# nianticlabs/implicit-depth

Hardware: AMD Instinct MI355X
Metric: frames/sec (BDModel.forward hot path, 512x384, 64 planes, 8-frame tuple = 1 current + 7 source views; third-party backbones excluded) (higher is better)
Workload: dtype f32

## Files before the change

### implicit-depth_amd/csrc/conv.hip

```cpp
#include <algorithm>
#include "conv_args.h"
#include "../../include/idh_ops.h"

using namespace idh_conv;

int idh_stem_op(const idh_op &op, hipStream_t st, bool launch);

namespace {

__device__ float g_zero_page[kZeroFloats];

thread_local bool t_dry_run = false;
thread_local int t_launches = 0;
#undef IDH_CHECK_LAUNCH
#define IDH_CHECK_LAUNCH()                                              \
    do {                                                                \
        if (!t_dry_run && hipGetLastError() != hipSuccess) return IDH_ELAUNCH; \
    } while (0)
#define IDH_LAUNCH(...)                         \
    do {                                        \
        if (t_dry_run) ++t_launches;            \
        else hipLaunchKernelGGL(__VA_ARGS__);   \
    } while (0)

// ... 694 lines not shown
        const int c4 = (int)(t & 3);
        long long r = t >> 2;
        const int co = (int)(r % Cout_pad);
        r /= Cout_pad;
        const int cq = (int)(r % (Cin_pad / 4));
        const int tap = (int)(r / (Cin_pad / 4));
        const int ci = cq * 4 + c4;
        float v = 0.f;
        if (ci < Cin && co < Cout) v = w[((size_t)co * Cin + ci) * taps + tap];
        dst[t] = v;
    }
}

__device__ __forceinline__ void upsample2_body(const float *__restrict__ in, float *__restrict__ out, int N, int H, int W, int C,
                                               int in_cs, int out_cs, unsigned blk, unsigned nblk) {
    const unsigned cq = (unsigned)C >> 2;
    const int Wo = 2 * W;
    const unsigned total = (unsigned)N * H * W * cq;
    constexpr float lo = 0.25f, hi = 0.75f;
    for (unsigned t = blk * 256u + threadIdx.x; t < total; t += nblk * 256u) {
        const unsigned q = t % cq;
        unsigned p = t / cq;
        const int ix = (int)(p % (unsigned)W);
        p /= (unsigned)W;
        const int iy = (int)(p % (unsigned)H);
        const int n = (int)(p / (unsigned)H);
        const int xm = max(ix - 1, 0), xp = min(ix + 1, W - 1);
        const int ym = max(iy - 1, 0), yp = min(iy + 1, H - 1);
        const float *b = in + (size_t)n * H * W * in_cs + 4 * q;
        const float *r0 = b + (size_t)ym * W * in_cs, *r1 = b + (size_t)iy * W * in_cs, *r2 = b + (size_t)yp * W * in_cs;
        float4 v[3][3];
        v[0][0] = *reinterpret_cast<const float4 *>(r0 + (size_t)xm * in_cs);
        v[0][1] = *reinterpret_cast<const float4 *>(r0 + (size_t)ix * in_cs);
        v[0][2] = *reinterpret_cast<const float4 *>(r0 + (size_t)xp * in_cs);
        v[1][0] = *reinterpret_cast<const float4 *>(r1 + (size_t)xm * in_cs);
        v[1][1] = *reinterpret_cast<const float4 *>(r1 + (size_t)ix * in_cs);
        v[1][2] = *reinterpret_cast<const float4 *>(r1 + (size_t)xp * in_cs);
        v[2][0] = *reinterpret_cast<const float4 *>(r2 + (size_t)xm * in_cs);
        v[2][1] = *reinterpret_cast<const float4 *>(r2 + (size_t)ix * in_cs);
        v[2][2] = *reinterpret_cast<const float4 *>(r2 + (size_t)xp * in_cs);
        float4 e[3], o[3];
#pragma unroll
        for (int r = 0; r < 3; ++r) {
            e[r].x = lo * v[r][0].x + hi * v[r][1].x; e[r].y = lo * v[r][0].y + hi * v[r][1].y;
            e[r].z = lo * v[r][0].z + hi * v[r][1].z; e[r].w = lo * v[r][0].w + hi * v[r][1].w;
            o[r].x = hi * v[r][1].x + lo * v[r][2].x; o[r].y = hi * v[r][1].y + lo * v[r][2].y;
            o[r].z = hi * v[r][1].z + lo * v[r][2].z; o[r].w = hi * v[r][1].w + lo * v[r][2].w;
        }
        float4 o00, o01, o10, o11;
        o00.x = lo * e[0].x + hi * e[1].x; o00.y = lo * e[0].y + hi * e[1].y; o00.z = lo * e[0].z + hi * e[1].z; o00.w = lo * e[0].w + hi * e[1].w;
        o01.x = lo * o[0].x + hi * o[1].x; o01.y = lo * o[0].y + hi * o[1].y; o01.z = lo * o[0].z + hi * o[1].z; o01.w = lo * o[0].w + hi * o[1].w;
        o10.x = hi * e[1].x + lo * e[2].x; o10.y = hi * e[1].y + lo * e[2].y; o10.z = hi * e[1].z + lo * e[2].z; o10.w = hi * e[1].w + lo * e[2].w;
        o11.x = hi * o[1].x + lo * o[2].x; o11.y = hi * o[1].y + lo * o[2].y; o11.z = hi * o[1].z + lo * o[2].z; o11.w = hi * o[1].w + lo * o[2].w;
        float *d = out + (((size_t)n * 2 * H + 2 * iy) * Wo + 2 * ix) * out_cs + 4 * q;
        *reinterpret_cast<float4 *>(d) = o00;
        *reinterpret_cast<float4 *>(d + out_cs) = o01;
        *reinterpret_cast<float4 *>(d + (size_t)Wo * out_cs) = o10;
        *reinterpret_cast<float4 *>(d + (size_t)Wo * out_cs + out_cs) = o11;
    }
}

__global__ __launch_bounds__(256) void upsample2_k(const float *__restrict__ in, float *__restrict__ out, int N, int H,
                                                   int W, int C, int in_cs, int out_cs) {
    upsample2_body(in, out, N, H, W, C, in_cs, out_cs, blockIdx.x, gridDim.x);
}

__global__ __launch_bounds__(256) void upsample2_nearest_k(const float *__restrict__ in, float *__restrict__ out, int N, int H,
                                                           int W, int C, int in_cs, int out_cs) {
    const int cq = C >> 2;
    const int Ho = 2 * H, Wo = 2 * W;
    const long long total = (long long)N * Ho * Wo * cq;
    for (long long t = blockIdx.x * 256ll + threadIdx.x; t < total; t += gridDim.x * 256ll) {
        const int q = (int)(t % cq);
        long long p = t / cq;
        const int x = (int)(p % Wo);
        p /= Wo;
        const int y = (int)(p % Ho);
        const int n = (int)(p / Ho);
        const float4 v = *reinterpret_cast<const float4 *>(in + (((size_t)n * H + (y >> 1)) * W + (x >> 1)) * in_cs + 4 * q);
        *reinterpret_cast<float4 *>(out + (((size_t)n * Ho + y) * Wo + x) * out_cs + 4 * q) = v;
    }
}

__global__ __launch_bounds__(256) void copy_nhwc_k(const float *__restrict__ in, float *__restrict__ out, long long npix, int C,
                                                   int in_cs, int out_cs) {
    const int cq = C >> 2;
    const long long total = npix * cq;
    for (long long t = blockIdx.x * 256ll + threadIdx.x; t < total; t += gridDim.x * 256ll) {
        const int q = (int)(t % cq);
        const long long p = t / cq;
        *reinterpret_cast<float4 *>(out + p * out_cs + 4 * q) = *reinterpret_cast<const float4 *>(in + p * in_cs + 4 * q);
    }
}

__device__ __forceinline__ void import_nchw_body(const float *__restrict__ src, float *__restrict__ dst, int C, int HW, int out_cs, int bx, int by, int img,
                                                 float (&tile)[32][65]) {
    const int p0 = bx * 64, c0 = by * 32;
    const float *s = src + (size_t)img * C * HW;
    float *d = dst + (size_t)img * HW * out_cs;
    for (int i = threadIdx.x; i < 64 * 32; i += 256) {
        const int p = i & 63, c = i >> 6;
        if (p0 + p < HW && c0 + c < C) tile[c][p] = s[(size_t)(c0 + c) * HW + p0 + p];
    }
    __syncthreads();
    for (int i = threadIdx.x; i < 64 * 32; i += 256) {
        const int c = i & 31, p = i >> 5;
        if (p0 + p < HW && c0 + c < C) d[(size_t)(p0 + p) * out_cs + c0 + c] = tile[c][p];
    }
}

__global__ __launch_bounds__(256) void import_nchw_k(const float *__restrict__ src, float *__restrict__ dst, int C,
                                                     int HW, int out_cs) {
    __shared__ float tile[32][65];
    import_nchw_body(src, dst, C, HW, out_cs, blockIdx.x, blockIdx.y, blockIdx.z, tile);
}

constexpr int kMaxImport = 8;
struct ImportGroupArgs {
    int n;
    unsigned start[kMaxImport + 1];
    struct { const float *src; float *dst; int C, HW, out_cs, nbx, nby; } d[kMaxImport];
};
__global__ __launch_bounds__(256) void import_nchw_group_k(const ImportGroupArgs g) {
    __shared__ float tile[32][65];
    int idx = 0;
    for (int i = 1; i < g.n; ++i)
        if (blockIdx.x >= g.start[i]) idx = i;
    const auto &m = g.d[idx];
    const unsigned local = blockIdx.x - g.start[idx];
    const int bx = (int)(local % (unsigned)m.nbx);
    const unsigned r = local / (unsigned)m.nbx;
    import_nchw_body(m.src, m.dst, m.C, m.HW, m.out_cs, bx, (int)(r % (unsigned)m.nby), (int)(r / (unsigned)m.nby), tile);
}

__global__ __launch_bounds__(256) void export_nchw_k(const float *__restrict__ src, float *__restrict__ dst, int C,
                                                     int HW, int in_cs) {
    __shared__ float tile[32][65];
    const int img = blockIdx.z;
    const int p0 = blockIdx.x * 64, c0 = blockIdx.y * 32;
    const float *s = src + (size_t)img * HW * in_cs;
    float *d = dst + (size_t)img * C * HW;
    for (int i = threadIdx.x; i < 64 * 32; i += 256) {
        const int c = i & 31, p = i >> 5;
        if (p0 + p < HW && c0 + c < C) tile[c][p] = s[(size_t)(p0 + p) * in_cs + c0 + c];
    }
    __syncthreads();
    for (int i = threadIdx.x; i < 64 * 32; i += 256) {
        const int p = i & 63, c = i >> 6;
        if (p0 + p < HW && c0 + c < C) d[(size_t)(c0 + c) * HW + p0 + p] = tile[c][p];
    }
}

constexpr int kPwCin = 64, kPwCout = 128, kPwTile = 64;
struct PwNchwArgs {
    const float *in, *w, *bias;
    float *out;
    int HW, out_cs, tiles_per_img;
    long long tiles;
};

__global__ __launch_bounds__(256, 4) void pointwise_nchw_k(const PwNchwArgs a) {
    constexpr int C16 = kPwCin / 16, NT = kPwCout / 16;
    __shared__ f32x4 sW[(kPwCin / 4) * kPwCout];
    {
        const f32x4 *g = reinterpret_cast<const f32x4 *>(a.w);
        for (int i = threadIdx.x; i < (kPwCin / 4) * kPwCout; i += 256) sW[i] = g[i];
    }
    __syncthreads();
    const int lane = threadIdx.x & 63;
    const int wave = __builtin_amdgcn_readfirstlane(threadIdx.x >> 6);
    const int ln = lane & 15, h = lane >> 4;

    const unsigned img_bytes = (unsigned)kPwCin * (unsigned)a.HW * 4u;
    auto load = [&](long long tile, f32x4 (&x)[C16]) {
        const int n = (int)(tile / a.tiles_per_img);
        const int p = (int)(tile - (long long)n * a.tiles_per_img) * kPwTile + 16 * wave + ln;
        const __amdgpu_buffer_rsrc_t rs = __builtin_amdgcn_make_buffer_rsrc(const_cast<float *>(a.in + (size_t)n * kPwCin * a.HW), 0, img_bytes, 0x00020000);
        const int voff = p < a.HW ? (4 * h * a.HW + p) * 4 : (int)0x7fffffff;
#pragma unroll
        for (int c = 0; c < C16; ++c)
#pragma unroll
            for (int e = 0; e < 4; ++e)
                x[c][e] = __builtin_bit_cast(float, __builtin_amdgcn_raw_buffer_load_b32(rs, voff, (16 * c + e) * a.HW * 4, 0));
    };
    auto compute = [&](long long tile, const f32x4 (&x)[C16]) {
        f32x4 acc[NT];
#pragma unroll
        for (int j = 0; j < NT; ++j) acc[j] = (f32x4){0.f, 0.f, 0.f, 0.f};
        int opaque = 0;
        asm volatile("" : "+s"(opaque));
        const f32x4 *sWt = sW + opaque;
#pragma unroll
        for (int c = 0; c < C16; ++c)
#pragma unroll
            for (int j = 0; j < NT; ++j) {
                const f32x4 A = sWt[(4 * c + h) * kPwCout + 16 * j + ln];
#pragma unroll
                for (int kk = 0; kk < 4; ++kk) acc[j] = __builtin_amdgcn_mfma_f32_16x16x4f32(A[kk], x[c][kk], acc[j], 0, 0, 0);
            }
        const int n = (int)(tile / a.tiles_per_img);
        const int p = (int)(tile - (long long)n * a.tiles_per_img) * kPwTile + 16 * wave + ln;
        if (p < a.HW) {
            float *o = a.out + ((size_t)n * a.HW + p) * a.out_cs + 4 * h;
#pragma unroll
            for (int j = 0; j < NT; ++j) {
                f32x4 v = acc[j];
                if (a.bias) v += *reinterpret_cast<const f32x4 *>(a.bias + 16 * j + 4 * h);
                *reinterpret_cast<f32x4 *>(o + 16 * j) = v;
            }
        }
    };
    f32x4 xa[C16], xb[C16];
    long long t = blockIdx.x;
    if (t >= a.tiles) return;
    load(t, xa);
    for (;;) {
        const long long t1 = t + gridDim.x;
        if (t1 < a.tiles) load(t1, xb);
        compute(t, xa);
        if (t1 >= a.tiles) break;
        const long long t2 = t1 + gridDim.x;
        if (t2 < a.tiles) load(t2, xa);
        compute(t1, xb);
        if (t2 >= a.tiles) break;
        t = t2;
    }
}

struct PwUpArgs {
    const float *in, *w, *bias, *low;
    float *out;
    int H, W, in_cs, low_cs, out_cs, tiles_per_img;
    long long tiles;
};

template <int C16, int NT>
__global__ __launch_bounds__(256) void pointwise_up_k(const PwUpArgs a) {
    constexpr int kCout = 16 * NT;
    extern __shared__ f32x4 sWu[];
    {
        const f32x4 *g = reinterpret_cast<const f32x4 *>(a.w);
        for (int i = threadIdx.x; i < 4 * C16 * kCout; i += 256) sWu[i] = g[i];
    }
    __syncthreads();
    const int lane = threadIdx.x & 63;
    const int wave = __builtin_amdgcn_readfirstlane(threadIdx.x >> 6);
    const int ln = lane & 15, h = lane >> 4;
    const int HW = a.H * a.W, Hl = a.H >> 1, Wl = a.W >> 1;
    for (long long tile = blockIdx.x; tile < a.tiles; tile += gridDim.x) {
        const int n = (int)(tile / a.tiles_per_img);
        const int p = (int)(tile - (long long)n * a.tiles_per_img) * kPwTile + 16 * wave + ln;
        const bool ok = p < HW;
        const int pc = ok ? p : 0;
        const float *ip = a.in + ((size_t)n * HW + pc) * a.in_cs + 4 * h;
        f32x4 x[C16];
#pragma unroll
        for (int c = 0; c < C16; ++c) x[c] = *reinterpret_cast<const f32x4 *>(ip + 16 * c);
        const int y = pc / a.W, xq = pc - y * a.W;
        const int iy = y >> 1, ix = xq >> 1;
        int y0, y1, x0, x1;
        float hy0, hy1, wx0, wx1;
        if (y & 1) { y0 = iy; y1 = min(iy + 1, Hl - 1); hy0 = 0.75f; hy1 = 0.25f; }
        else { y0 = max(iy - 1, 0); y1 = iy; hy0 = 0.25f; hy1 = 0.75f; }
        if (xq & 1) { x0 = ix; x1 = min(ix + 1, Wl - 1); wx0 = 0.75f; wx1 = 0.25f; }
        else { x0 = max(ix - 1, 0); x1 = ix; wx0 = 0.25f; wx1 = 0.75f; }
        const float *lb = a.low + (size_t)n * Hl * Wl * a.low_cs + 4 * h;
        const float *t00 = lb + ((size_t)y0 * Wl + x0) * a.low_cs, *t01 = lb + ((size_t)y0 * Wl + x1) * a.low_cs;
        const float *t10 = lb + ((size_t)y1 * Wl + x0) * a.low_cs, *t11 = lb + ((size_t)y1 * Wl + x1) * a.low_cs;
        f32x4 acc[NT];
#pragma unroll
        for (int j = 0; j < NT; ++j) acc[j] = a.bias ? *reinterpret_cast<const f32x4 *>(a.bias + 16 * j + 4 * h) : (f32x4){0.f, 0.f, 0.f, 0.f};
        int opaque = 0;
        asm volatile("" : "+s"(opaque));
        const f32x4 *sWt = sWu + opaque;
#pragma unroll
        for (int c = 0; c < C16; ++c)
#pragma unroll
            for (int j = 0; j < NT; ++j) {
                const f32x4 A = sWt[(4 * c + h) * kCout + 16 * j + ln];
#pragma unroll
                for (int kk = 0; kk < 4; ++kk) acc[j] = __builtin_amdgcn_mfma_f32_16x16x4f32(A[kk], x[c][kk], acc[j], 0, 0, 0);
            }
        if (ok) {
            float *o = a.out + ((size_t)n * HW + p) * a.out_cs + 4 * h;
#pragma unroll
            for (int j = 0; j < NT; ++j) {
                const f32x4 p00 = *reinterpret_cast<const f32x4 *>(t00 + 16 * j), p01 = *reinterpret_cast<const f32x4 *>(t01 + 16 * j);
                const f32x4 p10 = *reinterpret_cast<const f32x4 *>(t10 + 16 * j), p11 = *reinterpret_cast<const f32x4 *>(t11 + 16 * j);
                f32x4 v;
#pragma unroll
                for (int e = 0; e < 4; ++e) v[e] = acc[j][e] + (hy0 * (wx0 * p00[e] + wx1 * p01[e]) + hy1 * (wx0 * p10[e] + wx1 * p11[e]));
                *reinterpret_cast<f32x4 *>(o + 16 * j) = v;
            }
        }
    }
}

__global__ __launch_bounds__(256) void pointwise_head_k(const float *__restrict__ in, const float *__restrict__ w,
                                                        const float *__restrict__ bias, float *__restrict__ out,
                                                        float *__restrict__ out_exp, long long M, int C, int in_cs) {
    for (long long m = blockIdx.x * 256ll + threadIdx.x; m < M; m += gridDim.x * 256ll) {
        const float4 *p = reinterpret_cast<const float4 *>(in + m * in_cs);
        const float4 *wv = reinterpret_cast<const float4 *>(w);
        float s = 0.f;
        for (int q = 0; q < (C >> 2); ++q) {
            const float4 a = p[q], b = wv[q];
            s = fmaf(a.x, b.x, s); s = fmaf(a.y, b.y, s); s = fmaf(a.z, b.z, s); s = fmaf(a.w, b.w, s);
        }
        const float v = s + (bias ? bias[0] : 0.f);
        out[m] = v;
        if (out_exp) out_exp[m] = expf(v);
    }
}

constexpr int kInChunk = 1024;

template <int SUB>
__global__ __launch_bounds__(1024) void instnorm_stats_k(const float *__restrict__ in, int cs, int C, int HW, int nchunks,
                                                         float *__restrict__ part) {
    extern __shared__ float red[];
    const int n = blockIdx.y, chunk = blockIdx.x;
    const int cq = C >> 2;
    const int q = threadIdx.x % cq;
    const int prow = threadIdx.x / cq, pstep = (int)blockDim.x / cq;
    const int rows = SUB * pstep;
    const int p0 = chunk * kInChunk, p1 = min(HW, p0 + kInChunk);
    const float4 pv = *reinterpret_cast<const float4 *>(in + (size_t)n * HW * cs + 4 * q);
    float s[SUB][4], ss[SUB][4];
#pragma unroll
    for (int u = 0; u < SUB; ++u)
#pragma unroll
        for (int e = 0; e < 4; ++e) s[u][e] = ss[u][e] = 0.f;
    for (int p = p0 + prow; p < p1; p += rows) {
#pragma unroll
        for (int u = 0; u < SUB; ++u) {
            const int pp = p + u * pstep;
            if (pp < p1) {
                const float4 v = *reinterpret_cast<const float4 *>(in + ((size_t)n * HW + pp) * cs + 4 * q);
                const float d0 = v.x - pv.x, d1 = v.y - pv.y, d2 = v.z - pv.z, d3 = v.w - pv.w;
                s[u][0] += d0; s[u][1] += d1; s[u][2] += d2; s[u][3] += d3;
                ss[u][0] = fmaf(d0, d0, ss[u][0]); ss[u][1] = fmaf(d1, d1, ss[u][1]); ss[u][2] = fmaf(d2, d2, ss[u][2]); ss[u][3] = fmaf(d3, d3, ss[u][3]);
            }
        }
    }
#pragma unroll
    for (int u = 0; u < SUB; ++u) {
        float *mine = red + ((size_t)(prow + u * pstep) * cq + q) * 8;
#pragma unroll
        for (int e = 0; e < 4; ++e) { mine[e] = s[u][e]; mine[4 + e] = ss[u][e]; }
    }
    __syncthreads();
    for (int t = threadIdx.x; t < 8 * cq; t += blockDim.x) {
        const int qq = t >> 3, e = t & 7;
        float a = 0.f;
        for (int r = 0; r < rows; ++r) a += red[(r * cq + qq) * 8 + e];
        part[((size_t)(n * nchunks + chunk) * 2 + (e >> 2)) * C + 4 * qq + (e & 3)] = a;
    }
}

__global__ __launch_bounds__(256) void instnorm_finalize_k(const float *__restrict__ part, const float *__restrict__ in, int cs, int C, int HW,
                                                           int nchunks, float *__restrict__ stats) {
    const int n = blockIdx.x;
    for (int c = threadIdx.x; c < C; c += 256) {
        float s = 0.f, ss = 0.f;
        for (int k = 0; k < nchunks; ++k) {
            const float *o = part + ((size_t)(n * nchunks + k) * 2) * C + c;
            s += o[0];
            ss += o[C];
        }
        const float ms = s / (float)HW;
        const float var = fmaxf(ss / (float)HW - ms * ms, 0.f);
        stats[(size_t)n * 2 * C + c] = in[(size_t)n * HW * cs + c] + ms;
        stats[(size_t)n * 2 * C + C + c] = 1.0f / sqrtf(var + 1e-5f);
    }
}

__global__ __launch_bounds__(256) void instnorm_apply_k(const float *__restrict__ in, int cs, float *__restrict__ out, int out_cs,
                                                        int C, int HW, long long total, const float *__restrict__ stats, int act,
// ... 332 lines not shown
                PreparedConv pcs[kMaxGroup];
                int kinds[kMaxGroup];
                int run = 0;
                for (int j = i; j < n && run < kMaxGroup; ++j) {
                    const idh_op &o = ops[j];
                    if (j > i && (op.group == 0 || o.group != op.group)) break;
                    PreparedConv &pc = pcs[run];
                    if (o.kind == IDH_OP_CONV) {
                        const int rc = prep_conv(o, pc);
                        if (rc != IDH_OK) return rc;
                        kinds[run] = level_kind(pc);
                    } else if (o.kind == IDH_OP_UPSAMPLE2) {
                        const int rc = check_upsample(o);
                        if (rc != IDH_OK) return rc;
                        const idh_conv_src &us = o.src[0];
                        pc = PreparedConv{};
                        ConvArgs &c = pc.la.c;
                        c.s[0].in = us.in; c.s[0].H = us.H; c.s[0].W = us.W; c.s[0].Cin = us.Cin; c.s[0].cs = us.cs;
                        c.out = o.out; c.out_cs = o.out_cs; c.M = o.N; c.S = 1;
                        pc.a = c;
                        const long long tot = (long long)o.N * 4 * us.H * us.W * (us.Cin >> 2);
                        const long long natural = idh_cdiv(tot, 256);
                        pc.blocks = (unsigned)std::min<long long>(idh_cdiv(tot / 4, 256), kLevelUpsampleBlocks);
                        kinds[run] = natural <= kLevelUpsampleNatural ? LV_UP2 : -1;
                    } else {
                        break;
                    }
                    ++run;
                }
                int cnt = 0;
                if (op.kind == IDH_OP_CONV && pcs[0].lds_rows == 4 && !pcs[0].norm && !pcs[0].s2) {
                    cnt = 1;
                    while (cnt < run && ops[i + cnt].kind == IDH_OP_CONV && pcs[cnt].lds_rows == 4 && pcs[cnt].nj == pcs[0].nj &&
                           (!pcs[cnt].up || pcs[0].nj == 4) && !pcs[cnt].norm && !pcs[cnt].s2)
                        ++cnt;
                }
                int mix = 0;
                while (mix < run && kinds[mix] >= 0 && pcs[mix].blocks <= kLevelMaxBlocks) ++mix;
                int wg = 0;
                if (op.kind == IDH_OP_CONV && pcs[0].lds_rows == 32) {
                    wg = 1;
                    while (wg < run && wg < wino_max_group() && ops[i + wg].kind == IDH_OP_CONV && pcs[wg].lds_rows == 32 &&
                           (pcs[wg].a.s[1].in != nullptr) == (pcs[0].a.s[1].in != nullptr))
                        ++wg;
                }
                int rc, used;
                if (wg > 1) {
                    if (t_dry_run) {
                        ++t_launches;
                        rc = IDH_OK;
                    } else {
                        const ConvArgs *as[kMaxGroup];
                        int ns[kMaxGroup];
                        for (int j = 0; j < wg; ++j) { as[j] = &pcs[j].a; ns[j] = pcs[j].n_img; }
                        rc = launch_conv_wino_group(as, ns, wg, st);
                        if (rc == IDH_EUNSUPPORTED) {
                            rc = IDH_OK;
                            for (int j = 0; j < wg && rc == IDH_OK; ++j) rc = launch_conv(pcs[j], st);
                        }
                    }
                    used = wg;
                } else if (mix > cnt && mix > 1) {
                    rc = launch_level(pcs, kinds, mix, st);
                    used = mix;
                } else if (cnt > 1) {
                    rc = launch_group(pcs, cnt, st);
                    used = cnt;
                } else if (op.kind == IDH_OP_CONV) {
                    rc = launch_conv(pcs[0], st);
                    if (rc == IDH_OK) rc = launch_reduces(pcs, 1, st);
                    used = 1;
                } else {
                    const long long quads = (long long)op.N * s.H * s.W * (s.Cin >> 2);
                    int grid = idh_cdiv(quads, 256);
                    if (grid > 32768) grid = 32768;
                    IDH_LAUNCH(upsample2_k, dim3(grid), dim3(256), 0, st, s.in, op.out, op.N, s.H, s.W, s.Cin, s.cs, op.out_cs);
                    IDH_CHECK_LAUNCH();
                    rc = IDH_OK;
                    used = 1;
                }
                if (rc != IDH_OK) return rc;
                i += used - 1;
                break;
            }
            case IDH_OP_UPSAMPLE2_NEAREST: {
                if (!s.in || !op.out || (s.Cin & 3) || (s.cs & 3) || (op.out_cs & 3) || op.N <= 0) return IDH_EINVAL;
                const long long tot = (long long)op.N * 4 * s.H * s.W * (s.Cin >> 2);
                int grid = idh_cdiv(tot, 256);
                if (grid > 8192) grid = 8192;
                IDH_LAUNCH(upsample2_nearest_k, dim3(grid), dim3(256), 0, st, s.in, op.out, op.N, s.H, s.W, s.Cin, s.cs, op.out_cs);
                IDH_CHECK_LAUNCH();
                break;
            }
            case IDH_OP_NCHW_TO_NHWC: {
                ImportGroupArgs g{};
                unsigned cursor = 0;
                int run = 0;
                for (int j = i; j < n && run < kMaxImport; ++j) {
                    const idh_op &o = ops[j];
                    if (o.kind != IDH_OP_NCHW_TO_NHWC || (j > i && (op.group == 0 || o.group != op.group))) break;
                    const idh_conv_src &os = o.src[0];
                    if (!os.in || !o.out || o.N <= 0 || o.N > 65535 || os.H <= 0 || os.W <= 0 || os.Cin <= 0) return IDH_EINVAL;
                    const int HWj = os.H * os.W;
                    const long long blocks = (long long)idh_cdiv(HWj, 64) * idh_cdiv(os.Cin, 32) * o.N;
                    if (blocks > kLevelMaxBlocks * 8ll || cursor + blocks >= (1ll << 31)) break;
                    g.d[run].src = os.in; g.d[run].dst = o.out; g.d[run].C = os.Cin; g.d[run].HW = HWj; g.d[run].out_cs = o.out_cs;
                    g.d[run].nbx = idh_cdiv(HWj, 64); g.d[run].nby = idh_cdiv(os.Cin, 32);
                    g.start[run] = cursor;
                    cursor += (unsigned)blocks;
                    ++run;
                }
                if (run > 1) {
                    g.n = run;
                    g.start[run] = cursor;
                    IDH_LAUNCH(import_nchw_group_k, dim3(cursor), dim3(256), 0, st, g);
                    IDH_CHECK_LAUNCH();
                    i += run - 1;
                    break;
                }
                if (!s.in || !op.out || op.N <= 0 || op.N > 65535) return IDH_EINVAL;
                const int HW = s.H * s.W;
                IDH_LAUNCH(import_nchw_k, dim3(idh_cdiv(HW, 64), idh_cdiv(s.Cin, 32), op.N), dim3(256), 0, st, s.in,
                                   op.out, s.Cin, HW, op.out_cs);
                IDH_CHECK_LAUNCH();
                break;
            }
            case IDH_OP_NHWC_TO_NCHW: {
                if (!s.in || !op.out || op.N <= 0 || op.N > 65535) return IDH_EINVAL;
                const int HW = s.H * s.W;
                IDH_LAUNCH(export_nchw_k, dim3(idh_cdiv(HW, 64), idh_cdiv(s.Cin, 32), op.N), dim3(256), 0, st, s.in,
                                   op.out, s.Cin, HW, s.cs);
                IDH_CHECK_LAUNCH();
                break;
            }
            case IDH_OP_POINTWISE_HEAD: {
                if (!s.in || !s.w || !op.out || (s.Cin & 3) || (s.cs & 3)) return IDH_EINVAL;
                const long long M = (long long)op.N * s.H * s.W;
                int grid = idh_cdiv(M, 256);
                if (grid > 8192) grid = 8192;
                IDH_LAUNCH(pointwise_head_k, dim3(grid), dim3(256), 0, st, s.in, s.w, op.bias, op.out, op.ws, M, s.Cin,
                                   s.cs);
                IDH_CHECK_LAUNCH();
                break;
            }
            case IDH_OP_POINTWISE_NCHW: {
                if (!s.in || !s.w || !op.out || op.N <= 0 || s.H <= 0 || s.W <= 0 || (op.out_cs & 3) || ((uintptr_t)op.out & 15) ||
                    (op.bias && ((uintptr_t)op.bias & 15)))
                    return IDH_EINVAL;
                if (s.Cin != kPwCin || op.Cout != kPwCout || op.out_cs < kPwCout || (long long)s.H * s.W * kPwCin * 4 >= (1ll << 31))
                    return IDH_EUNSUPPORTED;
                PwNchwArgs pa{};
                pa.in = s.in; pa.w = s.w; pa.bias = op.bias; pa.out = op.out;
                pa.HW = s.H * s.W; pa.out_cs = op.out_cs;
                pa.tiles_per_img = idh_cdiv(pa.HW, kPwTile);
                pa.tiles = (long long)op.N * pa.tiles_per_img;
                const int grid = (int)std::min<long long>(pa.tiles, 256 * 4 * 4);
                IDH_LAUNCH(pointwise_nchw_k, dim3(grid), dim3(256), 0, st, pa);
                IDH_CHECK_LAUNCH();
                break;
            }
            case IDH_OP_POINTWISE_UP: {
                const idh_conv_src &lo = op.src[1];
                if (!s.in || !s.w || !lo.in || !op.out || op.N <= 0 || s.H <= 0 || s.W <= 0 || (s.H & 1) || (s.W & 1) || (s.cs & 3) || (lo.cs & 3) || (op.out_cs & 3) ||
                    s.cs < s.Cin || lo.cs < op.Cout || op.out_cs < op.Cout || ((uintptr_t)s.in & 15) || ((uintptr_t)lo.in & 15) || ((uintptr_t)op.out & 15) ||
                    ((uintptr_t)s.w & 15) || (op.bias && ((uintptr_t)op.bias & 15)) || lo.H != s.H / 2 || lo.W != s.W / 2)
                    return IDH_EINVAL;
                if (s.Cin != op.Cout || (s.Cin != 64 && s.Cin != 128) || (long long)s.H * s.W >= (1ll << 31)) return IDH_EUNSUPPORTED;
                PwUpArgs pa{};
                pa.in = s.in; pa.w = s.w; pa.bias = op.bias; pa.low = lo.in; pa.out = op.out;
                pa.H = s.H; pa.W = s.W; pa.in_cs = s.cs; pa.low_cs = lo.cs; pa.out_cs = op.out_cs;
                pa.tiles_per_img = idh_cdiv(s.H * s.W, kPwTile);
                pa.tiles = (long long)op.N * pa.tiles_per_img;
                const int grid = (int)std::min<long long>(pa.tiles, 256 * 8);
                if (s.Cin == 64) IDH_LAUNCH((pointwise_up_k<4, 4>), dim3(grid), dim3(256), 16 * 64 * sizeof(f32x4), st, pa);
                else IDH_LAUNCH((pointwise_up_k<8, 8>), dim3(grid), dim3(256), 32 * 128 * sizeof(f32x4), st, pa);
                IDH_CHECK_LAUNCH();
                break;
            }
            case IDH_OP_STEM: {
                const int rc = idh_stem_op(op, st, !t_dry_run);
                if (rc != IDH_OK) return rc;
                if (t_dry_run) ++t_launches;
                break;
            }
            case IDH_OP_COPY: {
                if (!s.in || !op.out || (s.Cin & 3) || (s.cs & 3) || (op.out_cs & 3) || op.N <= 0) return IDH_EINVAL;
                const long long npix = (long long)op.N * s.H * s.W;
                int grid = idh_cdiv(npix * (s.Cin >> 2), 256);
                if (grid > 8192) grid = 8192;
                IDH_LAUNCH(copy_nhwc_k, dim3(grid), dim3(256), 0, st, s.in, op.out, npix, s.Cin, s.cs, op.out_cs);
                IDH_CHECK_LAUNCH();
                break;
            }
            case IDH_OP_INSTNORM: {
                const int C = s.Cin, HW = s.H * s.W;
                if (!s.in || !op.ws || C <= 0 || (C & 3) || 256 % (C >> 2) || (s.cs & 3) || (op.out && (op.out_cs & 3)) ||
                    op.N <= 0 || op.N > 65535)
                    return IDH_EINVAL;
                const int nchunks = idh_cdiv(HW, kInChunk);
                const int sthreads = ((long long)nchunks * op.N < 512 && C >= 64) ? 1024 : 256;
                if (C >= 64 && sthreads == 256)
                    IDH_LAUNCH(instnorm_stats_k<4>, dim3(nchunks, op.N), dim3(256), 1024 * 8 * sizeof(float), st, s.in, s.cs, C, HW, nchunks, op.ws);
                else
                    IDH_LAUNCH(instnorm_stats_k<1>, dim3(nchunks, op.N), dim3(sthreads), sthreads * 8 * sizeof(float), st, s.in, s.cs, C, HW,
                                       nchunks, op.ws);
                IDH_CHECK_LAUNCH();
                float *stats = op.ws + (size_t)op.N * nchunks * 2 * C;
                IDH_LAUNCH(instnorm_finalize_k, dim3(op.N), dim3(256), 0, st, op.ws, s.in, s.cs, C, HW, nchunks, stats);
                IDH_CHECK_LAUNCH();
                if (!op.out) break;
                const long long total = (long long)op.N * HW * (C >> 2);
                int gx = idh_cdiv(total, 256 * 4);
                if (gx > 16384) gx = 16384;
                IDH_LAUNCH(instnorm_apply_k, dim3(gx), dim3(256), 0, st, s.in, s.cs, op.out, op.out_cs, C, HW, total, stats, op.act,
                                   op.slope);
                IDH_CHECK_LAUNCH();
                break;
            }
            default:
                return IDH_EINVAL;
        }
    }
    return IDH_OK;
}

extern "C" int idh_conv_variant(const idh_op *op, int32_t out[8]) {
    if (!op || !out || op->kind != IDH_OP_CONV) return IDH_EINVAL;
    PreparedConv pc{};
    const int rc = prep_conv(*op, pc);
    if (rc != IDH_OK) return rc;
    const bool lds = pc.lds_rows == 8 || pc.lds_rows == 4;
    out[0] = pc.lds_rows;
    out[1] = lds ? pc.nj : 0;
    out[2] = lds ? 0 : pc.tm;
    out[3] = lds ? 0 : pc.tn;
    out[4] = pc.a.S;
    out[5] = pc.up;
    out[6] = pc.norm;
    out[7] = pc.s2;
    return IDH_OK;
}

extern "C" int idh_count_launches(const idh_op *ops, int n) {
    t_dry_run = true;
    t_launches = 0;
    const int rc = idh_run_ops(ops, n, nullptr);
    t_dry_run = false;
    return rc == IDH_OK ? t_launches : rc;
}
```

Measured before the change: 690.9.

## Widen pointwise NCHW kernel to two pixels per lane with LDS-staged coalesced stores

The NCHW pointwise kernel now has each lane process two adjacent pixels, loaded with 64-bit buffer loads when alignment permits, which doubles the tile per wave. Accumulators are transposed through a swizzled per-wave LDS stage so output rows are written as contiguous 128-bit buffer stores, with bias read from LDS. Tile indexing moves to 32-bit and the occupancy hint drops from 4 to 3. The aim is fewer, wider memory transactions and better store coalescing, at the cost of higher register pressure and extra LDS traffic and wave barriers.

```diff
diff --git a/implicit-depth_amd/csrc/conv.hip b/implicit-depth_amd/csrc/conv.hip
--- a/implicit-depth_amd/csrc/conv.hip
+++ b/implicit-depth_amd/csrc/conv.hip
@@ -870,78 +870,116 @@
 }
 
 constexpr int kPwCin = 64, kPwCout = 128, kPwTile = 64;
+constexpr int kPwWaves = 4, kPwNchwTile = 32 * kPwWaves;
+typedef float f32x2 __attribute__((ext_vector_type(2)));
+typedef unsigned u32x4 __attribute__((ext_vector_type(4)));
 struct PwNchwArgs {
     const float *in, *w, *bias;
     float *out;
-    int HW, out_cs, tiles_per_img;
-    long long tiles;
+    int HW, out_cs;
+    unsigned tiles_per_img, tiles;
 };
 
-__global__ __launch_bounds__(256, 4) void pointwise_nchw_k(const PwNchwArgs a) {
+template <bool WIDE>
+__global__ __launch_bounds__(64 * kPwWaves, 3) void pointwise_nchw_k(const PwNchwArgs a) {
     constexpr int C16 = kPwCin / 16, NT = kPwCout / 16;
     __shared__ f32x4 sW[(kPwCin / 4) * kPwCout];
+    __shared__ f32x4 sStage[kPwWaves][16 * 8];
+    __shared__ f32x4 sBias[kPwCout / 4];
     {
         const f32x4 *g = reinterpret_cast<const f32x4 *>(a.w);
-        for (int i = threadIdx.x; i < (kPwCin / 4) * kPwCout; i += 256) sW[i] = g[i];
-    }
+        for (int i = threadIdx.x; i < (kPwCin / 4) * kPwCout; i += 64 * kPwWaves) sW[i] = g[i];
+    }
+    if (threadIdx.x < kPwCout / 4)
+        sBias[threadIdx.x] = a.bias ? reinterpret_cast<const f32x4 *>(a.bias)[threadIdx.x] : (f32x4){-0.f, -0.f, -0.f, -0.f};
     __syncthreads();
     const int lane = threadIdx.x & 63;
     const int wave = __builtin_amdgcn_readfirstlane(threadIdx.x >> 6);
     const int ln = lane & 15, h = lane >> 4;
+    const int l8 = lane & 7, r8 = lane >> 3;
+    f32x4 *stage = sStage[wave];
 
     const unsigned img_bytes = (unsigned)kPwCin * (unsigned)a.HW * 4u;
-    auto load = [&](long long tile, f32x4 (&x)[C16]) {
-        const int n = (int)(tile / a.tiles_per_img);
-        const int p = (int)(tile - (long long)n * a.tiles_per_img) * kPwTile + 16 * wave + ln;
+    constexpr int kOut = 0x7ffffff8;
+    auto load = [&](unsigned tile, f32x4 (&x)[2][C16]) {
+        const bool live = tile < a.tiles;
+        const unsigned n = live ? tile / a.tiles_per_img : 0u;
+        const int p = live ? (int)(tile - n * a.tiles_per_img) * kPwNchwTile + 32 * wave + 2 * ln : a.HW;
         const __amdgpu_buffer_rsrc_t rs = __builtin_amdgcn_make_buffer_rsrc(const_cast<float *>(a.in + (size_t)n * kPwCin * a.HW), 0, img_bytes, 0x00020000);
-        const int voff = p < a.HW ? (4 * h * a.HW + p) * 4 : (int)0x7fffffff;
+        const int voff = p < a.HW ? (4 * h * a.HW + p) * 4 : kOut;
+        const int voff1 = p + 1 < a.HW ? voff + 4 : kOut;
 #pragma unroll
         for (int c = 0; c < C16; ++c)
 #pragma unroll
-            for (int e = 0; e < 4; ++e)
-                x[c][e] = __builtin_bit_cast(float, __builtin_amdgcn_raw_buffer_load_b32(rs, voff, (16 * c + e) * a.HW * 4, 0));
+            for (int e = 0; e < 4; ++e) {
+                const int soff = (16 * c + e) * a.HW * 4;
+                if constexpr (WIDE) {
+                    const f32x2 v = __builtin_bit_cast(f32x2, __builtin_amdgcn_raw_buffer_load_b64(rs, voff, soff, 0));
+                    x[0][c][e] = v[0];
+                    x[1][c][e] = v[1];
+                } else {
+                    x[0][c][e] = __builtin_bit_cast(float, __builtin_amdgcn_raw_buffer_load_b32(rs, voff, soff, 0));
+                    x[1][c][e] = __builtin_bit_cast(float, __builtin_amdgcn_raw_buffer_load_b32(rs, voff1, soff, 0));
+                }
+            }
     };
-    auto compute = [&](long long tile, const f32x4 (&x)[C16]) {
-        f32x4 acc[NT];
-#pragma unroll
-        for (int j = 0; j < NT; ++j) acc[j] = (f32x4){0.f, 0.f, 0.f, 0.f};
-        int opaque = 0;
-        asm volatile("" : "+s"(opaque));
-        const f32x4 *sWt = sW + opaque;
-#pragma unroll
-        for (int c = 0; c < C16; ++c)
-#pragma unroll
-            for (int j = 0; j < NT; ++j) {
-                const f32x4 A = sWt[(4 * c + h) * kPwCout + 16 * j + ln];
-#pragma unroll
-                for (int kk = 0; kk < 4; ++kk) acc[j] = __builtin_amdgcn_mfma_f32_16x16x4f32(A[kk], x[c][kk], acc[j], 0, 0, 0);
-            }
-        const int n = (int)(tile / a.tiles_per_img);
-        const int p = (int)(tile - (long long)n * a.tiles_per_img) * kPwTile + 16 * wave + ln;
-        if (p < a.HW) {
-            float *o = a.out + ((size_t)n * a.HW + p) * a.out_cs + 4 * h;
-#pragma unroll
-            for (int j = 0; j < NT; ++j) {
-                f32x4 v = acc[j];
-                if (a.bias) v += *reinterpret_cast<const f32x4 *>(a.bias + 16 * j + 4 * h);
-                *reinterpret_cast<f32x4 *>(o + 16 * j) = v;
-            }
-        }
+    auto wave_sync = [] {
+        __builtin_amdgcn_fence(__ATOMIC_RELEASE, "wavefront");
+        __builtin_amdgcn_wave_barrier();
+        __builtin_amdgcn_fence(__ATOMIC_ACQUIRE, "wavefront");
     };
-    f32x4 xa[C16], xb[C16];
-    long long t = blockIdx.x;
-    if (t >= a.tiles) return;
+    auto compute = [&](unsigned tile, const f32x4 (&x)[2][C16]) {
+        const unsigned n = tile / a.tiles_per_img;
+        const int pw = (int)(tile - n * a.tiles_per_img) * kPwNchwTile + 32 * wave;
+        const int npix = min(max(a.HW - pw, 0), 32);
+        const unsigned long long ob = (unsigned long long)(a.out + ((size_t)n * a.HW + pw) * a.out_cs);
+        const unsigned ob_lo = (unsigned)__builtin_amdgcn_readfirstlane((int)(unsigned)ob), ob_hi = (unsigned)__builtin_amdgcn_readfirstlane((int)(unsigned)(ob >> 32));
+        float *obase = reinterpret_cast<float *>((unsigned long long)ob_lo | ((unsigned long long)ob_hi << 32));
+        const __amdgpu_buffer_rsrc_t ro = __builtin_amdgcn_make_buffer_rsrc(obase, 0, __builtin_amdgcn_readfirstlane(npix * a.out_cs * 4), 0x00020000);
+#pragma unroll
+        for (int s = 0; s < 2; ++s) {
+            f32x4 acc[NT];
+#pragma unroll
+            for (int j = 0; j < NT; ++j) acc[j] = (f32x4){0.f, 0.f, 0.f, 0.f};
+            int opaque = 0;
+            asm volatile("" : "+s"(opaque));
+            const f32x4 *sWt = sW + opaque;
+#pragma unroll
+            for (int c = 0; c < C16; ++c)
+#pragma unroll
+                for (int j = 0; j < NT; ++j) {
+                    const f32x4 A = sWt[(4 * c + h) * kPwCout + 16 * j + ln];
+#pragma unroll
+                    for (int kk = 0; kk < 4; ++kk) acc[j] = __builtin_amdgcn_mfma_f32_16x16x4f32(A[kk], x[s][c][kk], acc[j], 0, 0, 0);
+                }
+#pragma unroll
+            for (int q = 0; q < 4; ++q) {
+                wave_sync();
+#pragma unroll
+                for (int jj = 0; jj < 2; ++jj) stage[ln * 8 + ((4 * jj + h) ^ (ln & 7))] = acc[2 * q + jj];
+                wave_sync();
+#pragma unroll
+                for (int k = 0; k < 2; ++k) {
+                    const int r = r8 + 8 * k;
+                    const f32x4 v = stage[r * 8 + (l8 ^ (r & 7))] + sBias[8 * q + l8];
+                    __builtin_amdgcn_raw_buffer_store_b128(__builtin_bit_cast(u32x4, v), ro, ((2 * r + s) * a.out_cs + 4 * l8 + 32 * q) * 4, 0, 0);
+                }
+            }
+        }
+    };
+    f32x4 xa[2][C16], xb[2][C16];
+    unsigned t = blockIdx.x;
+    const unsigned step = gridDim.x;
     load(t, xa);
     for (;;) {
-        const long long t1 = t + gridDim.x;
-        if (t1 < a.tiles) load(t1, xb);
+        load(t + step, xb);
         compute(t, xa);
-        if (t1 >= a.tiles) break;
-        const long long t2 = t1 + gridDim.x;
-        if (t2 < a.tiles) load(t2, xa);
-        compute(t1, xb);
-        if (t2 >= a.tiles) break;
-        t = t2;
+        t += step;
+        if (t >= a.tiles) break;
+        load(t + step, xa);
+        compute(t, xb);
+        t += step;
+        if (t >= a.tiles) break;
     }
 }
 
@@ -1580,10 +1618,13 @@
                 PwNchwArgs pa{};
                 pa.in = s.in; pa.w = s.w; pa.bias = op.bias; pa.out = op.out;
                 pa.HW = s.H * s.W; pa.out_cs = op.out_cs;
-                pa.tiles_per_img = idh_cdiv(pa.HW, kPwTile);
-                pa.tiles = (long long)op.N * pa.tiles_per_img;
-                const int grid = (int)std::min<long long>(pa.tiles, 256 * 4 * 4);
-                IDH_LAUNCH(pointwise_nchw_k, dim3(grid), dim3(256), 0, st, pa);
+                const long long tiles = (long long)op.N * idh_cdiv(pa.HW, kPwNchwTile);
+                if (tiles >= (1ll << 31) || (long long)op.out_cs * 32 * 4 >= (1ll << 31)) return IDH_EUNSUPPORTED;
+                pa.tiles_per_img = (unsigned)idh_cdiv(pa.HW, kPwNchwTile);
+                pa.tiles = (unsigned)tiles;
+                const int grid = (int)std::min<long long>(tiles, 256 * 3 * 4);
+                if (!(pa.HW & 1) && !((uintptr_t)s.in & 7)) IDH_LAUNCH(pointwise_nchw_k<true>, dim3(grid), dim3(64 * kPwWaves), 0, st, pa);
+                else IDH_LAUNCH(pointwise_nchw_k<false>, dim3(grid), dim3(64 * kPwWaves), 0, st, pa);
                 IDH_CHECK_LAUNCH();
                 break;
             }
```

After: 694.7, median of 6. Within noise of the previous version (+0.6%).
